# JokerJohn/DCReg

Hardware: AMD Instinct MI355X
Metric: ICP iterations/sec (higher is better)
Workload: dtype f64

## Files before the change

### dcreg_amd/api.py

```python
import ctypes as C
import math
import os

import numpy as np

_HERE = os.path.dirname(os.path.abspath(__file__))
LIB_PATH = os.environ.get("DCREG_LIB") or os.path.join(_HERE, "lib", "libdcreg_hip.so")

DETECTION = {"NONE_DETE": 0, "SCHUR_CONDITION_NUMBER": 1, "FULL_EVD_MIN_EIGENVALUE": 2,
             "EVD_SUB_CONDITION": 3, "FULL_SVD_CONDITION": 4}
HANDLING = {"NONE_HAND": 0, "STANDARD_REGULARIZATION": 1, "ADAPTIVE_REGULARIZATION": 2,
            "PRECONDITIONED_CG": 3, "SOLUTION_REMAPPING": 4, "TRUNCATED_SVD": 5}
METHODS = {
    "ME-SR": ("FULL_EVD_MIN_EIGENVALUE", "SOLUTION_REMAPPING"),
    "ME-TSVD": ("FULL_EVD_MIN_EIGENVALUE", "TRUNCATED_SVD"),
    "ME-TReg": ("FULL_EVD_MIN_EIGENVALUE", "STANDARD_REGULARIZATION"),
    "FCN-SR": ("FULL_SVD_CONDITION", "SOLUTION_REMAPPING"),
    "Ours": ("SCHUR_CONDITION_NUMBER", "PRECONDITIONED_CG"),
    "NONE": ("NONE_DETE", "NONE_HAND"),
}

OK, E_INVALID, E_NOMEM, E_DEVICE, E_STATE = 0, -1, -2, -3, -4


# ... 89 lines not shown
_STRUCTS = {"dcreg_lin_params": LinParams, "dcreg_lin_out": LinOut, "dcreg_lin_debug": LinDebug,
            "dcreg_index_info": IndexInfo, "dcreg_config": Config, "dcreg_analysis": Analysis,
            "dcreg_iter_log": IterLog, "dcreg_icp_result": IcpResult, "dcreg_trial_result": TrialResult,
            "dcreg_launch_stats": LaunchStats, "dcreg_method_stats": MethodStats}

REDUCE_FN = C.CFUNCTYPE(C.c_int, C.POINTER(C.c_double), C.c_void_p)

EXPORTS = [
    "dcreg_backend_create", "dcreg_backend_destroy", "dcreg_last_error", "dcreg_set_stream", "dcreg_set_option",
    "dcreg_set_target", "dcreg_set_target_device", "dcreg_set_source", "dcreg_set_source_device",
    "dcreg_target_insert", "dcreg_target_insert_device", "dcreg_target_insert_source", "dcreg_target_crop", "dcreg_target_get",
    "dcreg_debug_index_check",
    "dcreg_default_lin_params", "dcreg_linearize", "dcreg_linearize_batch", "dcreg_linearize_batch_begin",
    "dcreg_linearize_batch_end", "dcreg_linearize_batch_begin_warm", "dcreg_reserve_warm_states", "dcreg_reset_warm_state", "dcreg_hint_misalignment", "dcreg_linearize_debug", "dcreg_launch_stats_get", "dcreg_knn", "dcreg_kdtree_build", "dcreg_kdtree_info", "dcreg_knn_timed",
    "dcreg_linearize_gated_begin", "dcreg_linearize_gate_open", "dcreg_linearize_gate_abort",
    "dcreg_index_info_get", "dcreg_kernel_time", "dcreg_launch_series", "dcreg_launch_series_passes", "dcreg_launch_series_structure", "dcreg_team_pass_stamps", "dcreg_roi_info", "dcreg_default_config", "dcreg_analyze_degeneracy", "dcreg_analyze_degeneracy_two_part",
    "dcreg_solve_degenerate_system", "dcreg_unpack_hessian", "dcreg_boxplus", "dcreg_pose6d_to_matrix",
    "dcreg_pose_error", "dcreg_icp_run", "dcreg_icp_run_sharded", "dcreg_icp_run_many", "dcreg_icp_run_euler", "dcreg_icp_run_trials", "dcreg_icp_run_montecarlo", "dcreg_p2p_error", "dcreg_sizeof", "dcreg_version", "dcreg_trial_pose",
    "dcreg_set_host_threads", "dcreg_get_host_threads", "dcreg_comm_unique_id", "dcreg_comm_init", "dcreg_comm_destroy", "dcreg_comm_allgather_sum", "dcreg_icp_run_sharded_rccl",
    "dcreg_montecarlo_job", "dcreg_comm_allgather", "dcreg_comm_info", "dcreg_set_error_message",
    "dcreg_register_frames", "dcreg_frames_load", "dcreg_frames_reserve_states", "dcreg_frames_reset_state", "dcreg_frames_batch_begin",
    "dcreg_register_pairs", "dcreg_pairs_plan", "dcreg_pairs_sources_load", "dcreg_pairs_build", "dcreg_pairs_reserve_states",
    "dcreg_pairs_reset_state", "dcreg_pairs_batch_begin",
    "dcreg_voxel_downsample", "dcreg_voxel_downsample_device", "dcreg_set_source_voxel", "dcreg_set_source_voxel_device",
    "dcreg_set_target_voxel", "dcreg_set_target_voxel_device",
    "dcreg_deskew", "dcreg_deskew_device", "dcreg_set_source_deskew", "dcreg_set_source_deskew_device",
    "dcreg_deskew_path", "dcreg_deskew_path_device", "dcreg_set_source_deskew_path", "dcreg_set_source_deskew_path_device",
    "dcreg_default_place_params", "dcreg_place_descriptors", "dcreg_place_descriptors_device", "dcreg_places_reset", "dcreg_places_count",
    "dcreg_places_add", "dcreg_places_add_clouds", "dcreg_places_add_clouds_device", "dcreg_places_add_source", "dcreg_places_get",
    "dcreg_places_query", "dcreg_places_query_clouds", "dcreg_places_query_clouds_device", "dcreg_places_query_source",
]
# ... 407 lines not shown
    L.dcreg_linearize_gated_begin.argtypes = [vp, C.c_int, C.POINTER(LinParams)]
    L.dcreg_linearize_gate_open.argtypes = [vp, dp, dp]
    L.dcreg_linearize_gate_abort.argtypes = [vp]
    L.dcreg_linearize_debug.argtypes = [vp, dp, dp, C.POINTER(LinParams), C.POINTER(LinOut), C.POINTER(LinDebug)]
    L.dcreg_knn.argtypes = [vp, fp, C.c_int64, C.c_int64, C.c_int, C.c_double, ip, fp]
    L.dcreg_kdtree_build.argtypes = [vp, C.c_int]
    L.dcreg_kdtree_info.argtypes = [vp, C.POINTER(C.c_int32), C.POINTER(C.c_int32), dp]
    L.dcreg_knn_timed.argtypes = [vp, fp, C.c_int64, C.c_int64, C.c_int, C.c_double, C.c_int, C.c_int, ip, fp, dp]
    L.dcreg_index_info_get.argtypes = [vp, C.POINTER(IndexInfo)]
    L.dcreg_kernel_time.argtypes = [vp, dp, C.POINTER(C.c_int64), C.c_int]
    L.dcreg_launch_series.argtypes = [vp, dp, C.POINTER(C.c_int64), C.POINTER(C.c_int64), C.POINTER(C.c_int64), C.c_int64, C.c_int]
    if hasattr(L, "dcreg_launch_series_passes"):
        L.dcreg_launch_series_passes.argtypes = [vp, C.POINTER(C.c_uint8), C.c_int64]
    if hasattr(L, "dcreg_launch_series_structure"):
        L.dcreg_launch_series_structure.argtypes = [vp, C.POINTER(C.c_uint8), C.c_int64]
    if hasattr(L, "dcreg_team_pass_stamps"):
        L.dcreg_team_pass_stamps.argtypes = [vp, C.POINTER(C.c_uint64), C.c_int64]
    L.dcreg_default_config.restype = None
    L.dcreg_default_config.argtypes = [C.POINTER(Config)]
    L.dcreg_analyze_degeneracy.argtypes = [dp, C.c_int, C.c_int, C.POINTER(Config), C.POINTER(Analysis)]
    L.dcreg_analyze_degeneracy_two_part.argtypes = [dp, C.c_int, C.c_int, C.POINTER(Config), C.POINTER(Analysis), C.POINTER(C.c_int)]
    L.dcreg_solve_degenerate_system.argtypes = [dp, dp, C.c_int, C.POINTER(Config), C.POINTER(Analysis), dp]
    L.dcreg_unpack_hessian.restype = None
    L.dcreg_unpack_hessian.argtypes = [dp, dp]
    L.dcreg_boxplus.restype = None
    L.dcreg_boxplus.argtypes = [dp, dp, dp, dp, dp]
    L.dcreg_pose6d_to_matrix.restype = None
    L.dcreg_pose6d_to_matrix.argtypes = [C.c_double] * 6 + [dp]
    L.dcreg_pose_error.restype = None
    L.dcreg_pose_error.argtypes = [dp, dp, dp, dp]
# ... 700 lines not shown

    def launch_series(self, reset=True, cap=1 << 20):
        lp = C.POINTER(C.c_int64)
        n = self._L.dcreg_launch_series(self._h, None, None, None, None, 0, 0)
        if n < 0:
            raise DcregError("dcreg_launch_series failed")
        n = min(n, cap)
        ms = np.empty(n, np.float64)
        se, rf, pt = np.empty(n, np.int64), np.empty(n, np.int64), np.empty(n, np.int64)
        adv = np.zeros(n, np.uint8)
        if hasattr(self._L, "dcreg_launch_series_passes"):
            self._L.dcreg_launch_series_passes(self._h, adv.ctypes.data_as(C.POINTER(C.c_uint8)), n)
        st = np.where((adv & 3) != 0, 1, 0).astype(np.uint8)
        if hasattr(self._L, "dcreg_launch_series_structure"):
            self._L.dcreg_launch_series_structure(self._h, st.ctypes.data_as(C.POINTER(C.c_uint8)), n)
        self._L.dcreg_launch_series(self._h, _dp(ms), se.ctypes.data_as(lp), rf.ctypes.data_as(lp), pt.ctypes.data_as(lp), n, int(reset))
        return {"ms": ms, "searched": se, "refitted": rf, "points": pt, "advanced": adv & 3, "one_wave": (adv >> 2) & 1, "structure": st}

    def team_pass_stamps(self):
        n = self._L.dcreg_team_pass_stamps(self._h, None, 0)
        if n <= 0:
            return np.zeros((0, 8), np.uint64)
        st = np.zeros((n + 1, 8), np.uint64)
        rc = self._L.dcreg_team_pass_stamps(self._h, st.ctypes.data_as(C.POINTER(C.c_uint64)), n + 1)
        if rc < 0:
            self._check(rc, "dcreg_team_pass_stamps")
        return st

    def roi_info(self):
        v = (C.c_double * 11)()
        self._L.dcreg_roi_info.argtypes = [C.c_void_p, C.POINTER(C.c_double)]
        self._check(self._L.dcreg_roi_info(self._h, v), "dcreg_roi_info")
# ... 226 lines not shown
```

### dcreg_amd/csrc/device/context.hip

```cpp
#include <algorithm>
#include <cmath>
#include <cstdarg>
#include <cstdio>
#include <cstdlib>
#include <chrono>
#include <cstring>
#include <string>
#include <vector>

#include <hip/hip_runtime.h>
#include <rocprim/device/device_radix_sort.hpp>
#include <rocprim/device/device_scan.hpp>

#include "../../../include/dcreg_debug.h"
#include "context.hpp"
#include "kernels.hpp"

namespace dcreg {

constexpr double kCountScale = 67108864.0;
constexpr size_t kSearchCountBytes = 64 * kCounterStride * sizeof(uint32_t);
static inline unsigned blocks_for(int64_t n, int bs) { return (unsigned)((n + bs - 1) / bs); }
static void drop_warm(dcreg_ctx *c);

// ... 1380 lines not shown
                                                    per_cell >= kTeamPassMinCellPts);
        P.pass = team ? LinPass::team : adv ? LinPass::advance : LinPass::none;
    }
    bool one_wave = false;
    if (L.n_poses > 1)
        one_wave = fused && !dbg && (c->opt_one_wave >= 2 || (c->opt_one_wave_batches && (uint64_t)L.n_poses * P.nbx >= (uint64_t)c->opt_one_wave_min_blocks));
    else if (!P.direct && !dbg && P.pass != LinPass::team) {
        const bool most = !L.uses_state(c) || fresh || !P.use_cert || (known && (double)c->last_searched >= c->opt_one_wave_min_frac * (double)L.n);
        one_wave = c->opt_one_wave >= 2 || (c->opt_one_wave == 1 && P.nbx >= (uint32_t)c->opt_one_wave_min_blocks && P.pass != LinPass::advance && most &&
                                            c->hint_misalign > c->opt_one_wave_min_cells * c->map.grid.h);
    }
    P.gate_inside = L.kind == LinKind::gated && c->opt_gate_in_kernel && P.nbx <= (uint32_t)kChunk && P.pass != LinPass::advance;
    P.body = (P.gate_inside && P.pass != LinPass::team) ? LinBody::gated : L.kind == LinKind::stamps ? LinBody::stamps : L.kind == LinKind::dump ? LinBody::dump :
             one_wave ? LinBody::one_wave : fused ? LinBody::fused : LinBody::chunked;
    P.pass_rows = P.pass == LinPass::advance && c->opt_advance_fused != 0 && !P.direct && P.body == LinBody::fused;
    return P;
}

static int stage_poses(dcreg_ctx *c, LinSlot &S, LinLaunch &L) {
    const int64_t n_states = L.frame_ids ? L.fs->n_states : c->n_batch_states;
    std::vector<uint8_t> &state_valid = L.frame_ids ? L.fs->state_valid : c->batch_state_valid;
    dcreg_ctx::StateKey &states_key = L.frame_ids ? L.fs->key : c->batch_state_key;
    const bool use_states = L.state_ids && c->opt_warm && n_states > 0;
    if (use_states && !(L.key == states_key)) {
        std::fill(state_valid.begin(), state_valid.end(), (uint8_t)0);
        states_key = L.key;
    }
    const int n_poses = L.n_poses;
    const size_t bytes = (size_t)n_poses * sizeof(PoseArg) + (L.frame_ids ? (size_t)n_poses * sizeof(uint2) : 0) +
                         (L.grid_ids ? (size_t)n_poses * sizeof(uint32_t) : 0);
// ... 141 lines not shown
    GateArgs gt{nullptr, nullptr, 0ull, nullptr, nullptr, 0u};
    const PoseArg *lin_poses = L.d_poses;
    if (gated) {
        const unsigned long long want = ++c->gate_seq;
        if (P.gate_inside) {
            gt = GateArgs{c->h_gate.dev(), c->d_gate_dev.data(), want, team ? c->d_gate_pose.data() : nullptr, team ? c->d_gate_abort.data() : nullptr, L.one.fresh};
            if (team) abort_flag = c->d_gate_abort.data();
            else lin_poses = nullptr;
        } else {
            hipLaunchKernelGGL(k_gate, dim3(1), dim3(64), 0, c->stream, c->h_gate.dev(), want, c->d_gate_pose.data(), L.one.fresh, c->d_gate_abort.data());
            abort_flag = c->d_gate_abort.data();
        }
    }
    if (int rc = record(S.ev0)) return rc;
    if (P.pass == LinPass::advance) {
        const auto pass = P.pass_rows ? k_advance<FAST, true> : k_advance<FAST, false>;
        hipLaunchKernelGGL(pass, dim3(blocks_for(L.n, kAdvTile)), dim3(kLinBlock), 0, c->stream, c->d_src.data(), n, c->map.grid, L.one, L.d_poses, L.a,
                           P.pass_rows ? nullptr : c->d_adv_counts.data(), abort_flag, S.d_partials.data(), P.nbx, fin);
    }
    if (team) {
        const auto pass = P.gate_inside ? k_advance_team<FAST, true> : k_advance_team<FAST>;
        hipLaunchKernelGGL(pass, dim3(blocks_for(L.n, kTeamTile)), dim3(kWave), 0, c->stream, c->d_src.data(), n, c->map.grid, L.one, P.gate_inside ? nullptr : L.d_poses,
                           L.a, c->d_adv_counts.data(), P.gate_inside ? nullptr : abort_flag, c->opt_team_stamps ? c->d_team_stamps.data() : nullptr, gt);
    }
    if (P.pass != LinPass::none) {
        if (int rc = bail(team ? "team advance pass launch" : "advance pass launch", hipGetLastError())) return rc;
        c->n_advance_launches += 1;
    }
    const bool one = P.one_wave(); const auto lin = lin_kernel<FAST>(P);
    if (!P.pass_rows)
    hipLaunchKernelGGL(lin, dim3(one ? P.nbx * (kLinBlock / kWave) : P.nbx, (unsigned)P.n_poses), dim3(one ? kWave : kLinBlock), 0, c->stream,
// ... 41 lines not shown
    LinLaunch L{slot, n_poses, R9, t3, state_ids, frame_ids, grid_ids, p, dbg_host, gated ? LinKind::gated : LinKind::single};
    if (int rc = lin_check(c, L)) return rc;
    if (c->need_set_device) { HIP_TRY(c, hipSetDevice(c->device)); }
    if (gated && c->roi_active && roi_pad_for(c, p->search_radius) > c->roi_pad) (void)roi_deactivate(c);
    if (!gated && L.kind != LinKind::pairs && (c->roi_active || roi_wanted(c))) {
        const bool product = L.kind == LinKind::single || L.kind == LinKind::stamps;
        if (int rc = product ? roi_ensure(c, L.R9, L.t3, p->search_radius) : roi_deactivate(c)) return rc;
    }
    L.a = make_lin_args(c, p, L.kind != LinKind::pairs, L.n);
    const LinArgs &a = L.a;
    L.key.radius_sq = a.radius_sq; L.key.max_thick_sq = a.max_thick_sq; L.key.min_norm = a.min_norm;
    L.key.radius_sq_f = a.radius_sq_f; L.key.cert_r_out = a.cert_r_out; L.key.cert_r_in = a.cert_r_in; L.key.fast_plane = c->opt_fast_plane ? 1 : 0;
    if (L.own() && !gated) {
        const double jump = c->last_pose_valid ? pose_jump(c, L.R9, L.t3, c->last_R, c->last_t) : 1e300;
        if (c->hint_unknown && jump <= 0.5 * c->map.grid.h) c->hint_misalign = c->hint_last;
        if (jump > 0.5 * c->map.grid.h) { c->last_searched = c->n_src; c->last_points = c->last_searched; }
        c->hint_unknown = false;
        std::memcpy(c->last_R, L.R9, sizeof(c->last_R)); std::memcpy(c->last_t, L.t3, sizeof(c->last_t));
        c->last_pose_valid = true;
    }
    if (!gated && order_wanted(c, L)) {
        bool stale = !c->order_valid;
        if (!stale && (int64_t)c->seq - c->est_launch >= 16)
            stale = pose_jump(c, L.R9, L.t3, c->est_R, c->est_t) > c->map.grid.h;
        if (int rc = stale ? estimate_dispatch_order(c, L.R9, L.t3, a.max_ring) : DCREG_OK) return rc;
    }
    if (L.uses_state(c) && !(L.key == c->state_key)) { c->state_valid = false; c->state_key = L.key; }
    L.state_was_valid = c->state_valid;
    L.one.state = kNoIdx; L.one.fresh = 1;
    if (L.own()) {
        std::memcpy(L.one.R, L.R9, sizeof(L.one.R)); std::memcpy(L.one.t, L.t3, sizeof(L.one.t));
// ... 115 lines not shown
        std::memcpy(outs[i].g, o + 21, 6 * sizeof(double));
        outs[i].sum_r2 = o[27]; outs[i].sum_b2 = o[28];
        int64_t c29 = (int64_t)std::llround(o[29]), c30 = (int64_t)std::llround(o[30]);
        if (coded) {
            const int64_t S26 = (int64_t)1 << 26;
            searched += c29 / S26; refitted += c30 / S26;
            c29 %= S26; c30 %= S26;
        }
        outs[i].n_eff = c29; outs[i].n_pt = c30;
    }
    c->last_points = (int64_t)P.n_poses * c->n_src;
    if (searched > c->last_points) searched = c->last_points;
    if (refitted > c->last_points) refitted = c->last_points;
    c->last_searched = searched; c->last_refitted = refitted;
    if (c->opt_record_launches && c->launch_series.size() < ((size_t)1 << 20))
        c->launch_series.push_back(dcreg_ctx::LaunchRec{(double)launch_ms, searched, refitted, c->last_points, P.passes(), P.structure()});
    return DCREG_OK;
}

int launch_linearize(dcreg_ctx *c, int n_poses, const double *R9, const double *t3, const dcreg_lin_params *p,
                     dcreg_lin_out *outs, dcreg_lin_debug *dbg_host) {
    if (c && !outs) { c->fail("null argument"); return DCREG_E_INVALID; }
    static const bool timing = std::getenv("DCREG_HOST_TIMING") != nullptr;
    using Clk = std::chrono::steady_clock;
    const auto t0 = Clk::now();
    int rc = linearize_begin(c, 0, n_poses, R9, t3, nullptr, p, dbg_host);
    if (rc) return rc;
    const auto t1 = Clk::now();
    rc = linearize_end(c, 0, outs);
    if (rc && c) c->slots[0].pending = false;
    if (timing && c) {
// ... 146 lines not shown
    else if (k == "roi_index") { c->opt_roi_index = (int)std::min(std::max(v, 0.0), 2.0); c->roi_built = false; }
    else if (k == "roi_margin") { c->opt_roi_margin = std::min(std::max(v, 0.0), 1.0e6); c->roi_built = false; }
    else if (k == "pair_max_table_entries") c->opt_pair_max_table_entries = (int64_t)std::min(std::max(v, 4096.0), 2147483648.0);
    else if (k == "pairs_max_bytes") c->opt_pairs_max_bytes = std::max(v, 0.0);
    else if (k == "max_table_entries") c->opt_max_table_entries = (int64_t)std::min(std::max(v, 1048576.0), 2147483648.0);
    else if (k == "advance") c->opt_advance = (int)v;
    else if (k == "advance_fused") c->opt_advance_fused = (int)v;
    else if (k == "one_wave") c->opt_one_wave = (int)v;
    else if (k == "one_wave_batches") c->opt_one_wave_batches = v != 0.0;
    else if (k == "one_wave_min_frac") c->opt_one_wave_min_frac = v;
    else if (k == "one_wave_min_cells") c->opt_one_wave_min_cells = v;
    else if (k == "one_wave_min_blocks") c->opt_one_wave_min_blocks = (int)v;
    else if (k == "gate_in_kernel") c->opt_gate_in_kernel = v != 0.0;
    else if (k == "team_stamps") c->opt_team_stamps = v != 0.0;
    else if (k == "team_pass") c->opt_team_pass = (int)v;
    else if (k == "advance_min_blocks") c->opt_advance_min_blocks = (int)v;
    else if (k == "team_search") c->opt_team_max = (int)v;
    else if (k == "spin") c->opt_spin = v != 0.0;
    else if (k == "far_bound") c->opt_far_bound = v != 0.0;
    else if (k == "dispatch_order") { c->opt_dispatch_order = v != 0.0; c->order_valid = false; }
    else if (k == "keep_source_order") c->opt_keep_source_order = v != 0.0;
    else if (k == "gap_field") c->opt_gap_field = v != 0.0;
    else if (k == "map_update") c->opt_map_update = v != 0.0 ? 1 : 0;
    else if (k == "map_grow_margin") c->opt_map_grow_margin = std::min(std::max(v, 0.0), 1.0e4);
    else { c->fail("unknown option '%s'", key); return DCREG_E_INVALID; }
    return DCREG_OK;
}

int dcreg_set_target(dcreg_ctx *c, const float *xyz, int64_t n, int64_t stride, double r) { return set_target(c, xyz, n, stride, r, false); }
int dcreg_set_target_device(dcreg_ctx *c, const float *xyz, int64_t n, int64_t stride, double r) { return set_target(c, xyz, n, stride, r, true); }
// ... 326 lines not shown

int dcreg_launch_series_passes(dcreg_ctx *c, uint8_t *advanced, int64_t cap) {
    if (!c || cap < 0) return -1;
    const int64_t n = std::min<int64_t>(cap, (int64_t)c->launch_series.size());
    for (int64_t i = 0; i < n; ++i) if (advanced) advanced[i] = (uint8_t)c->launch_series[(size_t)i].advanced;
    return (int)std::min<int64_t>((int64_t)c->launch_series.size(), 0x7FFFFFFF);
}

int dcreg_launch_series_structure(dcreg_ctx *c, uint8_t *structure, int64_t cap) {
    if (!c || cap < 0) return -1;
    const int64_t n = std::min<int64_t>(cap, (int64_t)c->launch_series.size());
    for (int64_t i = 0; i < n; ++i) if (structure) structure[i] = (uint8_t)c->launch_series[(size_t)i].structure;
    return (int)std::min<int64_t>((int64_t)c->launch_series.size(), 0x7FFFFFFF);
}

int dcreg_team_pass_stamps(dcreg_ctx *c, uint64_t *out, int64_t cap_blocks) {
    if (!c || cap_blocks < 0) return -1;
    if (!c->d_team_stamps || c->team_stamps_n == 0) return 0;
    const int64_t n = std::min<int64_t>(cap_blocks, (int64_t)c->team_stamps_n + 1);
    if (out && n > 0) {
        if (int rc = refuse_in_flight(c)) return rc;
        HIP_TRY(c, hipMemcpyAsync(out, c->d_team_stamps.data(), sizeof(unsigned long long) * 8 * (size_t)n, hipMemcpyDeviceToHost, c->stream));
        HIP_TRY(c, hipStreamSynchronize(c->stream));
    }
    return (int)std::min<int64_t>((int64_t)c->team_stamps_n, 0x7FFFFFFF);
}

int dcreg_kernel_time(dcreg_ctx *c, double *ms_total, int64_t *launches, int reset) {
    if (!c) return DCREG_E_INVALID;
    if (ms_total) *ms_total = c->kernel_ms_total;
// ... 7 lines not shown
```

### dcreg_amd/csrc/device/context.hpp

```cpp
#pragma once
#include <hip/hip_runtime.h>

#include <algorithm>
#include <chrono>
#include <cstdint>
#include <utility>
#include <vector>

#include "../../../include/dcreg.h"
#include "kernels.hpp"

struct dcreg_lin_params;
struct dcreg_lin_out;
struct dcreg_lin_debug;

#define HIP_TRY(ctx, expr)                                                                       \
    do {                                                                                         \
        hipError_t e__ = (expr);                                                                 \
        if (e__ != hipSuccess) {                                                                 \
            (ctx)->fail("%s failed: %s (%s:%d)", #expr, hipGetErrorString(e__), __FILE__, __LINE__); \
            return DCREG_E_DEVICE;                                                               \
        }                                                                                        \
    } while (0)

// ... 81 lines not shown
    }
    return (uint32_t)lo;
}
}

enum class LinKind : uint8_t { batch, frames, pairs, single, gated, dump, stamps };
enum class LinPass : uint8_t { none, advance, team };
enum class LinBody : uint8_t { chunked, fused, one_wave, gated, dump, stamps };
struct LinPlan {
    LinKind kind = LinKind::single; LinPass pass = LinPass::none; LinBody body = LinBody::fused;
    int n_poses = 0; uint32_t nbx = 0, n_chunks = 0;
    size_t n_rows = 0;
    bool direct = false;
    bool gate_inside = false;
    bool pass_rows = false;
    bool ordered = false, use_cert = true;
    bool fused() const { return body != LinBody::chunked; }
    bool one_wave() const { return body == LinBody::one_wave; }
    int passes() const { return (int)pass | (one_wave() ? 4 : 0); }
    int structure() const { return pass_rows ? 2 : pass != LinPass::none ? 1 : 0; }
};

struct LinSlot {
    DevBuf<double> d_partials;
    PinnedBuf<unsigned char> h_poses;
    DevBuf<unsigned char> d_poses;
    PinnedBuf<double> h_out;
    std::vector<double> h_rows;
    DevBuf<unsigned int> d_tickets;
    bool tickets_dirty = false;
// ... 199 lines not shown
    uint32_t group_blocks = 0, n_groups = 0;
    int n_cus = 256;
    void *kd = nullptr;
    bool order_valid = false;
    bool order_uneven = false;
    double est_R[9] = {}, est_t[3] = {};
    int64_t est_launch = 0;
    double hint_misalign = 1e300;
    bool hint_unknown = false;
    double hint_last = 1e300, last_R[9] = {}, last_t[3] = {};
    bool last_pose_valid = false;
    double opt_curve_x_scale = 1.0;
    int64_t opt_max_table_entries = (int64_t)1 << 30;
    int opt_advance = 1;
    int opt_advance_fused = 1;
    int opt_advance_min_blocks = 2048;
    int opt_team_pass = 1;
    bool opt_team_stamps = false;
    DevBuf<unsigned long long> d_team_stamps; uint32_t team_stamps_n = 0;
    DevBuf<uint32_t> d_adv_counts; bool adv_counts_dirty = true;
    int64_t n_advance_launches = 0;
    int opt_team_max = 7;
    bool opt_warm = true;
    int64_t n_launches = 0, n_poses_launched = 0, n_points_launched = 0;
    double kernel_ms_total = 0.0;
    int64_t kernel_launches = 0;
    int64_t last_searched = -1, last_refitted = -1, last_points = 0;
    struct LaunchRec { double ms; int64_t searched, refitted, points; int advanced, structure; };
    bool opt_record_launches = false;
    std::vector<LaunchRec> launch_series;

    void fail(const char *fmt, ...);
};

template <typename T>
int DevBuf<T>::ensure(dcreg_ctx *c, size_t need, const char *why) {
    if (holds(need)) return DCREG_OK;
    const size_t n = std::max<size_t>(need, 1);
    const hipError_t e = alloc(n);
    if (e != hipSuccess) {
        (void)hipGetLastError();
        if (why) c->fail("hipMalloc(%zu B) failed %s", n * sizeof(T), why);
        else c->fail("hipMalloc(%zu B) failed: %s", n * sizeof(T), hipGetErrorString(e));
// ... 71 lines not shown
```

### dcreg_amd/csrc/device/kernels.hpp

```cpp
#pragma once
#include <hip/hip_runtime.h>
#include <stdint.h>
#include <type_traits>

#include "search.hpp"

namespace dcreg {

template <int CTRL, int ROW_MASK>
__device__ __forceinline__ double dpp_add(double v) {
    const uint64_t b = (uint64_t)__double_as_longlong(v);
    int lo = (int)(uint32_t)b, hi = (int)(uint32_t)(b >> 32);
    lo = __builtin_amdgcn_update_dpp(0, lo, CTRL, ROW_MASK, 0xF, ROW_MASK == 0xF);
    hi = __builtin_amdgcn_update_dpp(0, hi, CTRL, ROW_MASK, 0xF, ROW_MASK == 0xF);
    const double o = __longlong_as_double((long long)(((uint64_t)(uint32_t)hi << 32) | (uint32_t)lo));
    return v + o;
}
__device__ __forceinline__ double wave_sum_to_lane63(double v) {
    v = dpp_add<0x111, 0xF>(v);
    v = dpp_add<0x112, 0xF>(v);
    v = dpp_add<0x114, 0xF>(v);
    v = dpp_add<0x118, 0xF>(v);
    v = dpp_add<0x142, 0xA>(v);
    v = dpp_add<0x143, 0xC>(v);
// ... 561 lines not shown
        if (threadIdx.x < kSlots) {
            double t = 0.0;
            if (threadIdx.x < 29) t = gm[gram_entry_of_slot(threadIdx.x)];
            else if (threadIdx.x < 31) t = cnt[0][threadIdx.x - 29];
            partials[(((size_t)pose_id * n_blocks_x + vb) * T + tile) * kSlots + threadIdx.x] = t;
        }
    } else {
    wave_rows_to_lds(row, flag, runs[wave].stage, &red[0][0] + wave * gm_stride, cnt, a.count_scale * (double)(w_search + adv_s),
                     a.count_scale * (double)(w_refit + adv_r));
    if constexpr (MODE == 2) stamp(5, __builtin_readcyclecounter());
    __syncthreads();
    block_publish<FUSED>(gm0, gm_stride, red, cnt, &s_role, partials + (size_t)pose_id * n_blocks_x * kSlots, vb, nb_pose, fin, pose_id);
    }
}

constexpr int kAdvDepth = 4;
constexpr int kAdvRowsBatch = 6;
static_assert((kAdvTile / kLinBlock) % kAdvRowsBatch == 0 && kAdvTile / kLinBlock <= kChunk, "whole batches; a tile spans at most two chunks");
template <bool FAST, bool ROWS = false>
static __global__ __launch_bounds__(kLinBlock, (kAdvDepth > 2 ? 2 : kLinOcc)) void k_advance(const float4 *__restrict__ src, uint32_t n_src, GridDev g, PoseArg pose1,
                                                                              const PoseArg *__restrict__ poses, LinArgs a,
                                                                              uint32_t *__restrict__ counts, const uint32_t *__restrict__ abort_flag,
                                                                              double *__restrict__ partials, uint32_t n_blocks_x, FinArgs fin) {
    if (abort_flag && *abort_flag != 0u) return;
    __shared__ RunList runs[kLinBlock / kWave];
    __shared__ uint16_t list[kAdvTile];
    __shared__ uint32_t n_list[2];
    __shared__ double red[kLinBlock / 32][kSlots];
    __shared__ double cnt[ROWS ? kAdvTile / kLinBlock : 1][kLinBlock / kWave][2];
    static_assert(sizeof(RunList) >= sizeof(double) * (kWave * kRowStride + (kAdvTile / kLinBlock) * 64), "a wave's Gram matrices of a tile live in its RunList");
    __shared__ uint32_t nofit[kAdvTile / 32];
    __shared__ int s_role;
    const int lane = threadIdx.x & 63, wave = threadIdx.x >> 6;
    PoseArg P;
    if (poses) P = poses[0]; else P = pose1;
    const size_t ss = a.state_stride;
    uint32_t *const sbase = a.state + (size_t)P.state * kStateRows * ss;
    typedef double dbl2 __attribute__((ext_vector_type(2)));
    uint4 *const SV0 = reinterpret_cast<uint4 *>(sbase + kStV0 * ss), *const SX = reinterpret_cast<uint4 *>(sbase + kStX * ss);
    dbl2 *const SV1 = reinterpret_cast<dbl2 *>(sbase + kStV1 * ss), *const SV2 = reinterpret_cast<dbl2 *>(sbase + kStV2 * ss);
    uint32_t *const SW3 = sbase + kStW3 * ss;
    uint2 *const SY = reinterpret_cast<uint2 *>(sbase + kStY * ss);
    if (threadIdx.x < 2) n_list[threadIdx.x] = 0u;
    if constexpr (ROWS) { if (threadIdx.x < (uint32_t)(kAdvTile / 32)) nofit[threadIdx.x] = 0u; }
    __syncthreads();
    const uint32_t base = blockIdx.x * (uint32_t)kAdvTile;
    constexpr int U = kAdvTile / kLinBlock;
    {
        float4 s4[U];
        uint4 v0[U];
        uint32_t w3[U];
#pragma unroll
        for (int u = 0; u < U; ++u) {
            const uint32_t i = base + (uint32_t)(u * kLinBlock) + threadIdx.x;
            const bool have = i < n_src;
            s4[u] = have ? src[i] : make_float4(0.f, 0.f, 0.f, 0.f);
            v0[u] = have ? SV0[i] : make_uint4(0x80000000u | 0x7F000000u, kFitNone, 0u, 0u);
            w3[u] = have ? SW3[i] : 0u;
        }
#pragma unroll
        for (int u = 0; u < U; ++u) {
            const uint32_t i = base + (uint32_t)(u * kLinBlock) + threadIdx.x;
            const bool have = i < n_src;
            float qx, qy, qz;
            body_to_global(P, (double)s4[u].x, (double)s4[u].y, (double)s4[u].z, qx, qy, qz);
            const float q0x = __uint_as_float(v0[u].z), q0y = __uint_as_float(v0[u].w), q0z = __uint_as_float(w3[u]);
            const bool need = have && !cert_holds(v0[u].x, q0x, q0y, q0z, qx, qy, qz);
            const bool refit = have && !need && !cert_is_out(v0[u].x) && !fit_holds(v0[u].y, q0x, q0y, q0z, qx, qy, qz);
            const unsigned long long ms = __builtin_amdgcn_ballot_w64(need), mr = __builtin_amdgcn_ballot_w64(refit);
            uint32_t bs = 0, br = 0;
            if (lane == 0) {
                if (ms) bs = atomicAdd(&n_list[0], (uint32_t)__builtin_popcountll(ms));
                if (mr) br = atomicAdd(&n_list[1], (uint32_t)__builtin_popcountll(mr));
            }
            bs = (uint32_t)__builtin_amdgcn_readfirstlane((int)bs); br = (uint32_t)__builtin_amdgcn_readfirstlane((int)br);
            const uint32_t ps = __builtin_amdgcn_mbcnt_hi((uint32_t)(ms >> 32), __builtin_amdgcn_mbcnt_lo((uint32_t)ms, 0u));
            const uint32_t pr = __builtin_amdgcn_mbcnt_hi((uint32_t)(mr >> 32), __builtin_amdgcn_mbcnt_lo((uint32_t)mr, 0u));
            const uint16_t off = (uint16_t)(u * kLinBlock + (int)threadIdx.x);
            if (need) list[bs + ps] = off;
            if (refit) list[(uint32_t)kAdvTile - 1u - (br + pr)] = off;
        }
    }
    __syncthreads();
    const uint32_t n_s = n_list[0], n_r = n_list[1];
    if (!ROWS && threadIdx.x == 0 && counts) { counts[(size_t)blockIdx.x * (kAdvTile / kLinBlock) * kCounterStride] = n_s; counts[(size_t)blockIdx.x * (kAdvTile / kLinBlock) * kCounterStride + 1] = n_r; }
    if (threadIdx.x == 0 && a.search_count && n_s)
        atomicAdd(a.search_count + (size_t)(blockIdx.x & 63u) * (kCounterStride / 2), (unsigned long long)n_s);
    const uint32_t c_s = (n_s + 63u) >> 6, c_r = (n_r + 63u) >> 6;
    auto chunk = [&](auto searching_c, uint32_t e, bool act) {
        constexpr bool searching = decltype(searching_c)::value;
        const uint32_t off = act ? (uint32_t)list[searching ? e : (uint32_t)kAdvTile - 1u - e] : 0u;
        const uint32_t i = base + off;
        const float4 s4 = src[i];
        float qx, qy, qz;
        body_to_global(P, (double)s4.x, (double)s4.y, (double)s4.z, qx, qy, qz);
// ... 33 lines not shown
                SV0[iw] = make_uint4(cert, fit.word, __float_as_uint(qx), __float_as_uint(qy));
                SV1[iw] = dbl2{fit.plane[0], fit.plane[1]};
                SV2[iw] = dbl2{fit.plane[2], fit.plane[3]};
                SW3[iw] = __float_as_uint(qz);
            }
        }
        if (act && !set) {
            SV0[iw] = make_uint4(cert, kFitNone, __float_as_uint(qx), __float_as_uint(qy));
            SW3[iw] = __float_as_uint(qz);
        }
    };
    for (uint32_t k = (uint32_t)wave; k < c_s; k += (uint32_t)(kLinBlock / kWave)) {
        const uint32_t e = k * 64u + (uint32_t)lane;
        chunk(std::true_type{}, e, e < n_s);
    }
    for (uint32_t k = ((uint32_t)wave + (uint32_t)(kLinBlock / kWave) - c_s % (uint32_t)(kLinBlock / kWave)) % (uint32_t)(kLinBlock / kWave); k < c_r;
         k += (uint32_t)(kLinBlock / kWave)) {
        const uint32_t e = k * 64u + (uint32_t)lane;
        chunk(std::false_type{}, e, e < n_r);
    }
    if constexpr (ROWS) {
        __syncthreads();
        const uint32_t vb0 = blockIdx.x * (uint32_t)U;
        const uint32_t nbt = min((uint32_t)U, n_blocks_x - vb0);
#pragma unroll
        for (int u0 = 0; u0 < U; u0 += kAdvRowsBatch) {
            if ((uint32_t)u0 >= nbt) break;
            float4 s4[kAdvRowsBatch];
            uint2 cf[kAdvRowsBatch];
            dbl2 p01[kAdvRowsBatch], p23[kAdvRowsBatch];
#pragma unroll
            for (int k = 0; k < kAdvRowsBatch; ++k) {
                const uint32_t i = base + (uint32_t)((u0 + k) * kLinBlock) + threadIdx.x;
                const bool have = i < n_src;
                s4[k] = have ? src[i] : make_float4(0.f, 0.f, 0.f, 0.f);
                cf[k] = have ? *reinterpret_cast<const uint2 *>(SV0 + i) : make_uint2(0x80000000u, kFitNone);
                p01[k] = have ? SV1[i] : dbl2{0.0, 0.0};
                p23[k] = have ? SV2[i] : dbl2{0.0, 0.0};
            }
#pragma unroll
            for (int k = 0; k < kAdvRowsBatch; ++k) {
                const int u = u0 + k;
                if ((uint32_t)u >= nbt) break;
                const uint32_t off = (uint32_t)(u * kLinBlock) + threadIdx.x;
                float qx, qy, qz;
                body_to_global(P, (double)s4[k].x, (double)s4[k].y, (double)s4[k].z, qx, qy, qz);
                uint8_t gate = 255;
                if (!cert_is_out(cf[k].x) && ((nofit[off >> 5] >> (off & 31u)) & 1u) == 0u) gate = (uint8_t)(cf[k].y & 3u);
                double nrm[3] = {0.0, 0.0, 0.0}, r_pt = 0.0, s_pt = 0.0;
                double row[8];
#pragma unroll
                for (int e = 0; e < 8; ++e) row[e] = 0.0;
                uint8_t flag = 0;
                if (base + off < n_src) {
                    const double plane[4] = {p01[k].x, p01[k].y, p23[k].x, p23[k].y};
                    if (gate == 0) flag = row_of_plane<FAST>(P, a, s4[k], qx, qy, qz, plane, row, nrm, r_pt, s_pt);
                    else flag = gate == 255 ? (uint8_t)0 : gate;
                }
                const bool first = u == 0 && wave == 0;
                wave_rows_to_lds(row, flag, runs[wave].stage, runs[wave].stage + kWave * kRowStride + u * 64, cnt[u], first ? a.count_scale * (double)n_s : 0.0,
                                 first ? a.count_scale * (double)n_r : 0.0);
            }
        }
        __syncthreads();
        if (threadIdx.x < nbt * (uint32_t)kSlots) {
            const uint32_t u = threadIdx.x / (uint32_t)kSlots, slot = threadIdx.x % (uint32_t)kSlots;
            double t = 0.0;
            if (slot < 29u) {
                const int e = gram_entry_of_slot((int)slot);
#pragma unroll
                for (int w = 0; w < kLinBlock / 64; ++w) t += (runs[w].stage + kWave * kRowStride)[u * 64u + (uint32_t)e];
            } else if (slot < 31u) {
#pragma unroll
                for (int w = 0; w < kLinBlock / 64; ++w) t += cnt[u][w][slot - 29u];
            }
            st_agent(partials + (size_t)(vb0 + u) * kSlots + slot, t);
            wait_stores();
        }
        __syncthreads();
        const uint32_t c0 = vb0 / kChunk;
        const uint32_t k0 = min(nbt, (c0 + 1u) * (uint32_t)kChunk - vb0), k1 = nbt - k0;
        const uint32_t cs0 = min((uint32_t)kChunk, n_blocks_x - c0 * kChunk);
        const uint32_t cs1 = k1 ? min((uint32_t)kChunk, n_blocks_x - (c0 + 1u) * kChunk) : 0u;
        if (threadIdx.x == 0) {
            unsigned int *const t0 = fin.tickets + (size_t)c0 * kCounterStride, *const t1 = t0 + kCounterStride;
            const unsigned int prev0 = __hip_atomic_fetch_add(t0, k0, __ATOMIC_RELAXED, __HIP_MEMORY_SCOPE_AGENT);
            unsigned int prev1 = 0u;
            if (k1) prev1 = __hip_atomic_fetch_add(t1, k1, __ATOMIC_RELAXED, __HIP_MEMORY_SCOPE_AGENT);
            const bool last0 = prev0 + k0 == cs0, last1 = k1 != 0u && prev1 + k1 == cs1;
// ... 1028 lines not shown
```

### include/dcreg_debug.h

```cpp
#ifndef DCREG_DEBUG_H
#define DCREG_DEBUG_H

#include "dcreg.h"

#ifdef __cplusplus
extern "C" {
#endif

typedef struct dcreg_lin_debug {
    int32_t *nn_idx;
    float *nn_d2;
    uint8_t *flag;
    double *normal;
    double *r;
    double *s;
    uint32_t *stats;
    uint64_t *stamps;
} dcreg_lin_debug;

int dcreg_linearize_debug(dcreg_ctx *, const double R[9], const double t[3], const dcreg_lin_params *,
                          dcreg_lin_out *, dcreg_lin_debug *);

int dcreg_kernel_time(dcreg_ctx *, double *ms_total, int64_t *launches, int reset);

typedef struct dcreg_launch_stats {
    int64_t launches;
    int64_t poses;
    int64_t points;
    int64_t points_searched;
    int64_t points_team;
} dcreg_launch_stats;
int dcreg_launch_stats_get(dcreg_ctx *, dcreg_launch_stats *, int reset);

int dcreg_launch_series(dcreg_ctx *, double *ms, int64_t *searched, int64_t *refitted, int64_t *points, int64_t cap, int reset);
int dcreg_launch_series_passes(dcreg_ctx *, uint8_t *advanced, int64_t cap);
int dcreg_launch_series_structure(dcreg_ctx *, uint8_t *structure, int64_t cap);

int dcreg_team_pass_stamps(dcreg_ctx *, uint64_t *out, int64_t cap_blocks);

int dcreg_roi_info(const dcreg_ctx *, double info[11]);

int dcreg_analyze_degeneracy_two_part(const double H[36], int detection, int handling, const dcreg_config *, dcreg_analysis *, int *owed);

int dcreg_kdtree_build(dcreg_ctx *, int leaf_size);
int dcreg_kdtree_info(const dcreg_ctx *, int32_t *depth, int32_t *leaf_size, double *build_ms);
int dcreg_knn_timed(dcreg_ctx *, const float *q_xyz, int64_t n, int64_t stride_floats, int k, double max_radius, int index, int repeats,
                    int32_t *idx, float *d2, double *kernel_ms);


int dcreg_frames_load(dcreg_ctx *, int n_frames, const float *xyz, const int64_t *frame_offsets, int64_t stride_floats);
int dcreg_frames_reserve_states(dcreg_ctx *, int64_t n_states);
// ... 21 lines not shown
```

Before: 16700.

## Add eager row-building variant of advance kernel for converged iterations

Adds an EAGER template form of k_advance that builds Hessian rows during the first certificate-check pass for tiles where no point needs search or refit. It loads the cached plane data alongside, so it can skip the second reload-and-rebuild pass and its barrier when nothing changed. By default it is only selected when the previous launch searched and refitted nothing, and the code also resets last_refitted on large pose jumps. The cost is extra register pressure and plane loads in the first pass, plus a smaller batch size, and the occupancy hint is raised.

```diff
diff --git a/dcreg_amd/api.py b/dcreg_amd/api.py
--- a/dcreg_amd/api.py
+++ b/dcreg_amd/api.py
@@ -127,7 +127,7 @@
     "dcreg_default_lin_params", "dcreg_linearize", "dcreg_linearize_batch", "dcreg_linearize_batch_begin",
     "dcreg_linearize_batch_end", "dcreg_linearize_batch_begin_warm", "dcreg_reserve_warm_states", "dcreg_reset_warm_state", "dcreg_hint_misalignment", "dcreg_linearize_debug", "dcreg_launch_stats_get", "dcreg_knn", "dcreg_kdtree_build", "dcreg_kdtree_info", "dcreg_knn_timed",
     "dcreg_linearize_gated_begin", "dcreg_linearize_gate_open", "dcreg_linearize_gate_abort",
-    "dcreg_index_info_get", "dcreg_kernel_time", "dcreg_launch_series", "dcreg_launch_series_passes", "dcreg_launch_series_structure", "dcreg_team_pass_stamps", "dcreg_roi_info", "dcreg_default_config", "dcreg_analyze_degeneracy", "dcreg_analyze_degeneracy_two_part",
+    "dcreg_index_info_get", "dcreg_kernel_time", "dcreg_launch_series", "dcreg_launch_series_passes", "dcreg_launch_series_structure", "dcreg_launch_series_eager", "dcreg_team_pass_stamps", "dcreg_roi_info", "dcreg_default_config", "dcreg_analyze_degeneracy", "dcreg_analyze_degeneracy_two_part",
     "dcreg_solve_degenerate_system", "dcreg_unpack_hessian", "dcreg_boxplus", "dcreg_pose6d_to_matrix",
     "dcreg_pose_error", "dcreg_icp_run", "dcreg_icp_run_sharded", "dcreg_icp_run_many", "dcreg_icp_run_euler", "dcreg_icp_run_trials", "dcreg_icp_run_montecarlo", "dcreg_p2p_error", "dcreg_sizeof", "dcreg_version", "dcreg_trial_pose",
     "dcreg_set_host_threads", "dcreg_get_host_threads", "dcreg_comm_unique_id", "dcreg_comm_init", "dcreg_comm_destroy", "dcreg_comm_allgather_sum", "dcreg_icp_run_sharded_rccl",
@@ -565,6 +565,8 @@
         L.dcreg_launch_series_passes.argtypes = [vp, C.POINTER(C.c_uint8), C.c_int64]
     if hasattr(L, "dcreg_launch_series_structure"):
         L.dcreg_launch_series_structure.argtypes = [vp, C.POINTER(C.c_uint8), C.c_int64]
+    if hasattr(L, "dcreg_launch_series_eager"):
+        L.dcreg_launch_series_eager.argtypes = [vp, C.POINTER(C.c_uint8), C.c_int64]
     if hasattr(L, "dcreg_team_pass_stamps"):
         L.dcreg_team_pass_stamps.argtypes = [vp, C.POINTER(C.c_uint64), C.c_int64]
     L.dcreg_default_config.restype = None
@@ -1295,8 +1297,11 @@
         st = np.where((adv & 3) != 0, 1, 0).astype(np.uint8)
         if hasattr(self._L, "dcreg_launch_series_structure"):
             self._L.dcreg_launch_series_structure(self._h, st.ctypes.data_as(C.POINTER(C.c_uint8)), n)
+        eg = np.zeros(n, np.uint8)
+        if hasattr(self._L, "dcreg_launch_series_eager"):
+            self._L.dcreg_launch_series_eager(self._h, eg.ctypes.data_as(C.POINTER(C.c_uint8)), n)
         self._L.dcreg_launch_series(self._h, _dp(ms), se.ctypes.data_as(lp), rf.ctypes.data_as(lp), pt.ctypes.data_as(lp), n, int(reset))
-        return {"ms": ms, "searched": se, "refitted": rf, "points": pt, "advanced": adv & 3, "one_wave": (adv >> 2) & 1, "structure": st}
+        return {"ms": ms, "searched": se, "refitted": rf, "points": pt, "advanced": adv & 3, "one_wave": (adv >> 2) & 1, "structure": st, "eager": eg}
 
     def team_pass_stamps(self):
         n = self._L.dcreg_team_pass_stamps(self._h, None, 0)
diff --git a/dcreg_amd/csrc/device/context.hip b/dcreg_amd/csrc/device/context.hip
--- a/dcreg_amd/csrc/device/context.hip
+++ b/dcreg_amd/csrc/device/context.hip
@@ -1418,6 +1418,9 @@
     P.body = (P.gate_inside && P.pass != LinPass::team) ? LinBody::gated : L.kind == LinKind::stamps ? LinBody::stamps : L.kind == LinKind::dump ? LinBody::dump :
              one_wave ? LinBody::one_wave : fused ? LinBody::fused : LinBody::chunked;
     P.pass_rows = P.pass == LinPass::advance && c->opt_advance_fused != 0 && !P.direct && P.body == LinBody::fused;
+    constexpr double kEagerMaxListed = 0.0;
+    const double listed = known ? (double)(c->last_searched + std::max<int64_t>(c->last_refitted, 0)) / (double)L.n : -1.0;
+    P.pass_eager = P.pass_rows && (c->opt_advance_eager >= 2 || (c->opt_advance_eager == 1 && known && listed <= kEagerMaxListed));
     return P;
 }
 
@@ -1589,7 +1592,7 @@
     }
     if (int rc = record(S.ev0)) return rc;
     if (P.pass == LinPass::advance) {
-        const auto pass = P.pass_rows ? k_advance<FAST, true> : k_advance<FAST, false>;
+        const auto pass = P.pass_eager ? k_advance<FAST, true, true> : P.pass_rows ? k_advance<FAST, true> : k_advance<FAST, false>;
         hipLaunchKernelGGL(pass, dim3(blocks_for(L.n, kAdvTile)), dim3(kLinBlock), 0, c->stream, c->d_src.data(), n, c->map.grid, L.one, L.d_poses, L.a,
                            P.pass_rows ? nullptr : c->d_adv_counts.data(), abort_flag, S.d_partials.data(), P.nbx, fin);
     }
@@ -1661,7 +1664,7 @@
     if (L.own() && !gated) {
         const double jump = c->last_pose_valid ? pose_jump(c, L.R9, L.t3, c->last_R, c->last_t) : 1e300;
         if (c->hint_unknown && jump <= 0.5 * c->map.grid.h) c->hint_misalign = c->hint_last;
-        if (jump > 0.5 * c->map.grid.h) { c->last_searched = c->n_src; c->last_points = c->last_searched; }
+        if (jump > 0.5 * c->map.grid.h) { c->last_searched = c->n_src; c->last_refitted = 0; c->last_points = c->last_searched; }
         c->hint_unknown = false;
         std::memcpy(c->last_R, L.R9, sizeof(c->last_R)); std::memcpy(c->last_t, L.t3, sizeof(c->last_t));
         c->last_pose_valid = true;
@@ -1807,7 +1810,7 @@
     if (refitted > c->last_points) refitted = c->last_points;
     c->last_searched = searched; c->last_refitted = refitted;
     if (c->opt_record_launches && c->launch_series.size() < ((size_t)1 << 20))
-        c->launch_series.push_back(dcreg_ctx::LaunchRec{(double)launch_ms, searched, refitted, c->last_points, P.passes(), P.structure()});
+        c->launch_series.push_back(dcreg_ctx::LaunchRec{(double)launch_ms, searched, refitted, c->last_points, P.passes(), P.structure(), P.pass_eager ? 1 : 0});
     return DCREG_OK;
 }
 
@@ -1984,6 +1987,7 @@
     else if (k == "gate_in_kernel") c->opt_gate_in_kernel = v != 0.0;
     else if (k == "team_stamps") c->opt_team_stamps = v != 0.0;
     else if (k == "team_pass") c->opt_team_pass = (int)v;
+    else if (k == "advance_eager") c->opt_advance_eager = (int)v;
     else if (k == "advance_min_blocks") c->opt_advance_min_blocks = (int)v;
     else if (k == "team_search") c->opt_team_max = (int)v;
     else if (k == "spin") c->opt_spin = v != 0.0;
@@ -2340,6 +2344,13 @@
     return (int)std::min<int64_t>((int64_t)c->launch_series.size(), 0x7FFFFFFF);
 }
 
+int dcreg_launch_series_eager(dcreg_ctx *c, uint8_t *eager, int64_t cap) {
+    if (!c || cap < 0) return -1;
+    const int64_t n = std::min<int64_t>(cap, (int64_t)c->launch_series.size());
+    for (int64_t i = 0; i < n; ++i) if (eager) eager[i] = (uint8_t)c->launch_series[(size_t)i].eager;
+    return (int)std::min<int64_t>((int64_t)c->launch_series.size(), 0x7FFFFFFF);
+}
+
 int dcreg_team_pass_stamps(dcreg_ctx *c, uint64_t *out, int64_t cap_blocks) {
     if (!c || cap_blocks < 0) return -1;
     if (!c->d_team_stamps || c->team_stamps_n == 0) return 0;
diff --git a/dcreg_amd/csrc/device/context.hpp b/dcreg_amd/csrc/device/context.hpp
--- a/dcreg_amd/csrc/device/context.hpp
+++ b/dcreg_amd/csrc/device/context.hpp
@@ -119,6 +119,7 @@
     bool direct = false;
     bool gate_inside = false;
     bool pass_rows = false;
+    bool pass_eager = false;
     bool ordered = false, use_cert = true;
     bool fused() const { return body != LinBody::chunked; }
     bool one_wave() const { return body == LinBody::one_wave; }
@@ -348,6 +349,7 @@
     int64_t opt_max_table_entries = (int64_t)1 << 30;
     int opt_advance = 1;
     int opt_advance_fused = 1;
+    int opt_advance_eager = 1;
     int opt_advance_min_blocks = 2048;
     int opt_team_pass = 1;
     bool opt_team_stamps = false;
@@ -360,7 +362,7 @@
     double kernel_ms_total = 0.0;
     int64_t kernel_launches = 0;
     int64_t last_searched = -1, last_refitted = -1, last_points = 0;
-    struct LaunchRec { double ms; int64_t searched, refitted, points; int advanced, structure; };
+    struct LaunchRec { double ms; int64_t searched, refitted, points; int advanced, structure, eager; };
     bool opt_record_launches = false;
     std::vector<LaunchRec> launch_series;
 
diff --git a/dcreg_amd/csrc/device/kernels.hpp b/dcreg_amd/csrc/device/kernels.hpp
--- a/dcreg_amd/csrc/device/kernels.hpp
+++ b/dcreg_amd/csrc/device/kernels.hpp
@@ -599,15 +599,18 @@
     }
 }
 
+constexpr int kAdvEagerBatch = 3;
 constexpr int kAdvDepth = 4;
 constexpr int kAdvRowsBatch = 6;
 static_assert((kAdvTile / kLinBlock) % kAdvRowsBatch == 0 && kAdvTile / kLinBlock <= kChunk, "whole batches; a tile spans at most two chunks");
-template <bool FAST, bool ROWS = false>
-static __global__ __launch_bounds__(kLinBlock, (kAdvDepth > 2 ? 2 : kLinOcc)) void k_advance(const float4 *__restrict__ src, uint32_t n_src, GridDev g, PoseArg pose1,
+static_assert((kAdvTile / kLinBlock) % kAdvEagerBatch == 0, "whole batches");
+template <bool FAST, bool ROWS = false, bool EAGER = false>
+static __global__ __launch_bounds__(kLinBlock, (EAGER && FAST ? 3 : kAdvDepth > 2 ? 2 : kLinOcc)) void k_advance(const float4 *__restrict__ src, uint32_t n_src, GridDev g, PoseArg pose1,
                                                                               const PoseArg *__restrict__ poses, LinArgs a,
                                                                               uint32_t *__restrict__ counts, const uint32_t *__restrict__ abort_flag,
                                                                               double *__restrict__ partials, uint32_t n_blocks_x, FinArgs fin) {
     if (abort_flag && *abort_flag != 0u) return;
+    static_assert(!EAGER || ROWS, "the eager form builds rows: it comes with ROWS");
     __shared__ RunList runs[kLinBlock / kWave];
     __shared__ uint16_t list[kAdvTile];
     __shared__ uint32_t n_list[2];
@@ -631,27 +634,36 @@
     __syncthreads();
     const uint32_t base = blockIdx.x * (uint32_t)kAdvTile;
     constexpr int U = kAdvTile / kLinBlock;
-    {
-        float4 s4[U];
-        uint4 v0[U];
-        uint32_t w3[U];
-#pragma unroll
-        for (int u = 0; u < U; ++u) {
-            const uint32_t i = base + (uint32_t)(u * kLinBlock) + threadIdx.x;
+    constexpr int TB = EAGER ? kAdvEagerBatch : U;
+    [[maybe_unused]] uint32_t dirty = 0u;
+#pragma unroll
+    for (int u0 = 0; u0 < U; u0 += TB) {
+        float4 s4[TB];
+        uint4 v0[TB];
+        uint32_t w3[TB];
+        [[maybe_unused]] dbl2 p01[EAGER ? TB : 1], p23[EAGER ? TB : 1];
+#pragma unroll
+        for (int k = 0; k < TB; ++k) {
+            const uint32_t i = base + (uint32_t)((u0 + k) * kLinBlock) + threadIdx.x;
             const bool have = i < n_src;
-            s4[u] = have ? src[i] : make_float4(0.f, 0.f, 0.f, 0.f);
-            v0[u] = have ? SV0[i] : make_uint4(0x80000000u | 0x7F000000u, kFitNone, 0u, 0u);
-            w3[u] = have ? SW3[i] : 0u;
-        }
-#pragma unroll
-        for (int u = 0; u < U; ++u) {
+            s4[k] = have ? src[i] : make_float4(0.f, 0.f, 0.f, 0.f);
+            v0[k] = have ? SV0[i] : make_uint4(0x80000000u | 0x7F000000u, kFitNone, 0u, 0u);
+            w3[k] = have ? SW3[i] : 0u;
+            if constexpr (EAGER) {
+                p01[k] = have ? SV1[i] : dbl2{0.0, 0.0};
+                p23[k] = have ? SV2[i] : dbl2{0.0, 0.0};
+            }
+        }
+#pragma unroll
+        for (int k = 0; k < TB; ++k) {
+            const int u = u0 + k;
             const uint32_t i = base + (uint32_t)(u * kLinBlock) + threadIdx.x;
             const bool have = i < n_src;
             float qx, qy, qz;
-            body_to_global(P, (double)s4[u].x, (double)s4[u].y, (double)s4[u].z, qx, qy, qz);
-            const float q0x = __uint_as_float(v0[u].z), q0y = __uint_as_float(v0[u].w), q0z = __uint_as_float(w3[u]);
-            const bool need = have && !cert_holds(v0[u].x, q0x, q0y, q0z, qx, qy, qz);
-            const bool refit = have && !need && !cert_is_out(v0[u].x) && !fit_holds(v0[u].y, q0x, q0y, q0z, qx, qy, qz);
+            body_to_global(P, (double)s4[k].x, (double)s4[k].y, (double)s4[k].z, qx, qy, qz);
+            const float q0x = __uint_as_float(v0[k].z), q0y = __uint_as_float(v0[k].w), q0z = __uint_as_float(w3[k]);
+            const bool need = have && !cert_holds(v0[k].x, q0x, q0y, q0z, qx, qy, qz);
+            const bool refit = have && !need && !cert_is_out(v0[k].x) && !fit_holds(v0[k].y, q0x, q0y, q0z, qx, qy, qz);
             const unsigned long long ms = __builtin_amdgcn_ballot_w64(need), mr = __builtin_amdgcn_ballot_w64(refit);
             uint32_t bs = 0, br = 0;
             if (lane == 0) {
@@ -664,6 +676,23 @@
             const uint16_t off = (uint16_t)(u * kLinBlock + (int)threadIdx.x);
             if (need) list[bs + ps] = off;
             if (refit) list[(uint32_t)kAdvTile - 1u - (br + pr)] = off;
+            if constexpr (EAGER) {
+                if ((ms | mr) != 0ull) dirty |= 1u << u;
+                else if ((uint32_t)u < min((uint32_t)U, n_blocks_x - blockIdx.x * (uint32_t)U)) {
+                    const uint8_t gate = cert_is_out(v0[k].x) ? (uint8_t)255 : (uint8_t)(v0[k].y & 3u);
+                    double nrm[3] = {0.0, 0.0, 0.0}, r_pt = 0.0, s_pt = 0.0;
+                    double row[8];
+#pragma unroll
+                    for (int e = 0; e < 8; ++e) row[e] = 0.0;
+                    uint8_t flag = 0;
+                    if (have) {
+                        const double plane[4] = {p01[k].x, p01[k].y, p23[k].x, p23[k].y};
+                        if (gate == 0) flag = row_of_plane<FAST>(P, a, s4[k], qx, qy, qz, plane, row, nrm, r_pt, s_pt);
+                        else flag = gate == 255 ? (uint8_t)0 : gate;
+                    }
+                    wave_rows_to_lds(row, flag, runs[wave].stage, runs[wave].stage + kWave * kRowStride + u * 64, cnt[u]);
+                }
+            }
         }
     }
     __syncthreads();
@@ -727,34 +756,39 @@
         const uint32_t e = k * 64u + (uint32_t)lane;
         chunk(std::true_type{}, e, e < n_s);
     }
+    if constexpr (EAGER) { if ((uint32_t)wave < c_s) dirty = (1u << U) - 1u; }
     for (uint32_t k = ((uint32_t)wave + (uint32_t)(kLinBlock / kWave) - c_s % (uint32_t)(kLinBlock / kWave)) % (uint32_t)(kLinBlock / kWave); k < c_r;
          k += (uint32_t)(kLinBlock / kWave)) {
         const uint32_t e = k * 64u + (uint32_t)lane;
         chunk(std::false_type{}, e, e < n_r);
     }
     if constexpr (ROWS) {
-        __syncthreads();
+        const bool rebuild = !EAGER || n_s + n_r != 0u;
+        if (rebuild) __syncthreads();
         const uint32_t vb0 = blockIdx.x * (uint32_t)U;
         const uint32_t nbt = min((uint32_t)U, n_blocks_x - vb0);
-#pragma unroll
-        for (int u0 = 0; u0 < U; u0 += kAdvRowsBatch) {
+        constexpr int RB = EAGER ? kAdvEagerBatch : kAdvRowsBatch;
+        if (rebuild) {
+#pragma unroll
+        for (int u0 = 0; u0 < U; u0 += RB) {
             if ((uint32_t)u0 >= nbt) break;
-            float4 s4[kAdvRowsBatch];
-            uint2 cf[kAdvRowsBatch];
-            dbl2 p01[kAdvRowsBatch], p23[kAdvRowsBatch];
-#pragma unroll
-            for (int k = 0; k < kAdvRowsBatch; ++k) {
+            float4 s4[RB];
+            uint2 cf[RB];
+            dbl2 p01[RB], p23[RB];
+#pragma unroll
+            for (int k = 0; k < RB; ++k) {
                 const uint32_t i = base + (uint32_t)((u0 + k) * kLinBlock) + threadIdx.x;
-                const bool have = i < n_src;
+                const bool have = i < n_src && (!EAGER || ((dirty >> (u0 + k)) & 1u) != 0u);
                 s4[k] = have ? src[i] : make_float4(0.f, 0.f, 0.f, 0.f);
                 cf[k] = have ? *reinterpret_cast<const uint2 *>(SV0 + i) : make_uint2(0x80000000u, kFitNone);
                 p01[k] = have ? SV1[i] : dbl2{0.0, 0.0};
                 p23[k] = have ? SV2[i] : dbl2{0.0, 0.0};
             }
 #pragma unroll
-            for (int k = 0; k < kAdvRowsBatch; ++k) {
+            for (int k = 0; k < RB; ++k) {
                 const int u = u0 + k;
                 if ((uint32_t)u >= nbt) break;
+                if constexpr (EAGER) { if (((dirty >> u) & 1u) == 0u) continue; }
                 const uint32_t off = (uint32_t)(u * kLinBlock) + threadIdx.x;
                 float qx, qy, qz;
                 body_to_global(P, (double)s4[k].x, (double)s4[k].y, (double)s4[k].z, qx, qy, qz);
@@ -770,10 +804,11 @@
                     if (gate == 0) flag = row_of_plane<FAST>(P, a, s4[k], qx, qy, qz, plane, row, nrm, r_pt, s_pt);
                     else flag = gate == 255 ? (uint8_t)0 : gate;
                 }
-                const bool first = u == 0 && wave == 0;
+                const bool first = !EAGER && u == 0 && wave == 0;
                 wave_rows_to_lds(row, flag, runs[wave].stage, runs[wave].stage + kWave * kRowStride + u * 64, cnt[u], first ? a.count_scale * (double)n_s : 0.0,
                                  first ? a.count_scale * (double)n_r : 0.0);
             }
+        }
         }
         __syncthreads();
         if (threadIdx.x < nbt * (uint32_t)kSlots) {
@@ -786,6 +821,7 @@
             } else if (slot < 31u) {
 #pragma unroll
                 for (int w = 0; w < kLinBlock / 64; ++w) t += cnt[u][w][slot - 29u];
+                if constexpr (EAGER) { if (u == 0u) t += a.count_scale * (double)(slot == 29u ? n_s : n_r); }
             }
             st_agent(partials + (size_t)(vb0 + u) * kSlots + slot, t);
             wait_stores();
diff --git a/include/dcreg_debug.h b/include/dcreg_debug.h
--- a/include/dcreg_debug.h
+++ b/include/dcreg_debug.h
@@ -35,6 +35,7 @@
 int dcreg_launch_series(dcreg_ctx *, double *ms, int64_t *searched, int64_t *refitted, int64_t *points, int64_t cap, int reset);
 int dcreg_launch_series_passes(dcreg_ctx *, uint8_t *advanced, int64_t cap);
 int dcreg_launch_series_structure(dcreg_ctx *, uint8_t *structure, int64_t cap);
+int dcreg_launch_series_eager(dcreg_ctx *, uint8_t *eager, int64_t cap);
 
 int dcreg_team_pass_stamps(dcreg_ctx *, uint64_t *out, int64_t cap_blocks);
 
```

Result: no change. 16630, median of 2 (-0.5%).
